# icdm-adteam/MoCoPCI

Hardware: AMD Instinct MI355X
Metric: interpolated frames/sec (higher is better)
Workload: dtype f32 (fused MLP layers: fp32 products as 6 bf16-MFMA partials of an exact 3-way split, fp32 accumulate; index paths exact f32)

## Files before the change

mocopci_amd/csrc/attention.hip:

```cpp
#include "attention_wide_fwd.h"

namespace {

typedef mcp_f2 f2;
constexpr int KT = 64;

template <int HD>
__global__ __launch_bounds__(64 * WAVES) void attention_small_kernel(int nq, int nk, int heads, const float *__restrict__ q, int qs,
                                                                     const float *__restrict__ k, int ks, const float *__restrict__ v,
                                                                     int vs, float scale_log2e, float *__restrict__ out, int os, int kv_shift) {
    constexpr int KS = HD + 1;
    __shared__ float kt[2][KT * KS];
    __shared__ __attribute__((aligned(16))) float vt[2][KT * HD];
    const int tid = threadIdx.x, lane = tid & 63, wave = tid >> 6, h = lane >> 5, col = lane & 31;
    const int head = blockIdx.y, bf = blockIdx.z;
    const int qi = blockIdx.x * (32 * WAVES) + wave * 32 + col;
    const bool live = qi < nq;
    q += ((size_t)bf * nq + (live ? qi : 0)) * qs + head * HD;
    int bkv = bf + kv_shift;
    if (bkv >= (int)gridDim.z) bkv -= (int)gridDim.z;
    k += (size_t)bkv * nk * ks + head * HD;
    v += (size_t)bkv * nk * vs + head * HD;

    float qf[HD / 2];
#pragma unroll
    for (int s = 0; s < HD / 2; ++s) qf[s] = q[2 * s + h] * scale_log2e;

    float m = -INFINITY, l = 0.f;
    f2 o[HD / 2];
#pragma unroll
    for (int d = 0; d < HD / 2; ++d) o[d] = f2{0.f, 0.f};

    constexpr int F4_PER_TILE = KT * HD / 4;
    constexpr int LOADS = (2 * F4_PER_TILE + 64 * WAVES - 1) / (64 * WAVES);
    float4 pre[LOADS];
    auto fetch = [&](int t) {
#pragma unroll
        for (int u = 0; u < LOADS; ++u) {
            const int e = tid + u * 64 * WAVES;
            const bool isv = e >= F4_PER_TILE;
            const int f = isv ? e - F4_PER_TILE : e;
            const int row = f / (HD / 4), c4 = f % (HD / 4);
            const int key = t * KT + row;
            pre[u] = make_float4(0.f, 0.f, 0.f, 0.f);
            if (e < 2 * F4_PER_TILE && key < nk) {
                const float *src = (isv ? v + (size_t)key * vs : k + (size_t)key * ks) + c4 * 4;
                pre[u] = *reinterpret_cast<const float4 *>(src);
            }
        }
    };
    auto stash = [&](int buf) {
#pragma unroll
        for (int u = 0; u < LOADS; ++u) {
            const int e = tid + u * 64 * WAVES;
            if (e >= 2 * F4_PER_TILE) continue;
            const bool isv = e >= F4_PER_TILE;
            const int f = isv ? e - F4_PER_TILE : e;
            const int row = f / (HD / 4), c4 = f % (HD / 4);
            if (isv) {
                *reinterpret_cast<float4 *>(&vt[buf][row * HD + c4 * 4]) = pre[u];
            } else {
                float *dst = &kt[buf][row * KS + c4 * 4];
                dst[0] = pre[u].x; dst[1] = pre[u].y; dst[2] = pre[u].z; dst[3] = pre[u].w;
            }
        }
    };

    const int stages = (nk + KT - 1) / KT;
    fetch(0);
    stash(0);
    for (int t = 0; t < stages; ++t) {
        const int cur = t & 1;
        if (t + 1 < stages) fetch(t + 1);
        __syncthreads();
#pragma unroll
        for (int sub = 0; sub < KT / 32; ++sub) {
            const float *ka = &kt[cur][(sub * 32 + col) * KS + h];
            f32x16 acc;
#pragma unroll
            for (int r = 0; r < 16; ++r) acc[r] = 0.f;
#pragma unroll
            for (int s = 0; s < HD / 2; ++s) acc = __builtin_amdgcn_mfma_f32_32x32x2f32(ka[2 * s], qf[s], acc, 0, 0, 0);
            const int kbase = t * KT + sub * 32;
            if (kbase + 32 > nk) {
#pragma unroll
                for (int r = 0; r < 16; ++r)
                    if (kbase + chan_of(r, h) >= nk) acc[r] = -INFINITY;
            }
            float mt = acc[0];
#pragma unroll
            for (int r = 1; r < 16; ++r) mt = fmaxf(mt, acc[r]);
            const float mn = fmaxf(m, mt);
            if (mn == -INFINITY) continue;
            const float alpha = __builtin_amdgcn_exp2f(m - mn);
            m = mn;
            l *= alpha;
            const f2 alpha2 = {alpha, alpha};
#pragma unroll
            for (int d = 0; d < HD / 2; ++d) o[d] = o[d] * alpha2;
#pragma unroll
            for (int r = 0; r < 16; ++r) {
                const float p = __builtin_amdgcn_exp2f(acc[r] - mn);
                l += p;
                const float *vr = &vt[cur][(sub * 32 + chan_of(r, h)) * HD];
                const f2 p2 = {p, p};
#pragma unroll
                for (int d = 0; d < HD; d += 4) {
                    const float4 vv = *reinterpret_cast<const float4 *>(vr + d);
                    o[d / 2 + 0] = mcp_f2_fma(p2, f2{vv.x, vv.y}, o[d / 2 + 0]);
                    o[d / 2 + 1] = mcp_f2_fma(p2, f2{vv.z, vv.w}, o[d / 2 + 1]);
                }
            }
        }
        if (t + 1 < stages) stash(cur ^ 1);
    }
    const float mo = __shfl_xor(m, 32), lo = __shfl_xor(l, 32);
    const float mm = fmaxf(m, mo);
    const float a0 = m == -INFINITY ? 0.f : __builtin_amdgcn_exp2f(m - mm), a1 = mo == -INFINITY ? 0.f : __builtin_amdgcn_exp2f(mo - mm);
    const float lsum = l * a0 + lo * a1;
    const float inv = 1.0f / lsum;
    float res[HD];
#pragma unroll
    for (int d = 0; d < HD; ++d) {
        const float od = (d & 1) ? o[d / 2].y : o[d / 2].x;
        res[d] = (od * a0 + __shfl_xor(od, 32) * a1) * inv;
    }
    if (live && h == 0) {
        float *dst = out + ((size_t)bf * nq + qi) * os + head * HD;
#pragma unroll
        for (int d = 0; d < HD; d += 4) *reinterpret_cast<float4 *>(dst + d) = make_float4(res[d], res[d + 1], res[d + 2], res[d + 3]);
    }
}

__device__ __forceinline__ int kv_batch(int kv_shift) {
    const int bkv = (int)blockIdx.z + kv_shift;
    return bkv >= (int)gridDim.z ? bkv - (int)gridDim.z : bkv;
}

template <int HD>
__global__ __launch_bounds__(64 * WAVES, 1) void attention_wide_kernel(int nq, int nk, const float *__restrict__ q, int qs,
                                                                       const float *__restrict__ k, int ks, const float *__restrict__ v,
                                                                       int vs, float scale_log2e, float *__restrict__ out, int os, int kv_shift) {
    extern __shared__ __attribute__((aligned(16))) float lds_w[];
    attention_wide_body<HD, false>(lds_w, nq, nk, (int)gridDim.y, q, qs, k, ks, v, vs, kv_batch(kv_shift), scale_log2e, 0, 0, 0.f, out, os, nullptr);
}

template <int HD>
__global__ __launch_bounds__(64 * WAVES, 1) void attention_wide_ksplit_kernel(int nq, int nk, const float *__restrict__ q, int qs,
                                                                              const float *__restrict__ k, int ks, const float *__restrict__ v,
                                                                              int vs, float scale_log2e, float *__restrict__ out, int os, int kv_shift) {
    extern __shared__ __attribute__((aligned(16))) float lds_ws[];
    attention_wide_ksplit_body<HD, false>(lds_ws, nq, nk, (int)gridDim.y, q, qs, k, ks, v, vs, kv_batch(kv_shift), scale_log2e, 0, 0, 0.f, out, os,
                                          nullptr);
}

template <int HD>
int launch_wide_ksplit(int bf, int nq, int nk, int heads, const float *q, int qs, const float *k, int ks, const float *v, int vs, float sl2,
                       float *out, int os, int kv_shift, hipStream_t s) {
    auto kern = attention_wide_ksplit_kernel<HD>;
    static McpPerDeviceOnce attr_once;
    if (attr_once.need()) {
        { const hipError_t attr_e_ = hipFuncSetAttribute(reinterpret_cast<const void *>(kern), hipFuncAttributeMaxDynamicSharedMemorySize, 160 * 1024); if (attr_e_ != hipSuccess) return (int)attr_e_; }
        attr_once.done();
    }
    hipLaunchKernelGGL(kern, dim3(mcp_divup(nq, 32), heads, bf), dim3(64 * WAVES), WideSplitCfg<HD>::LDS_BYTES, s, nq, nk, q, qs, k, ks, v, vs, sl2,
                       out, os, kv_shift);
    return mcp_launch_status();
}

template <int HD>
int launch_wide(int bf, int nq, int nk, int heads, const float *q, int qs, const float *k, int ks, const float *v, int vs, float sl2,
                float *out, int os, int kv_shift, hipStream_t s) {
    auto kern = attention_wide_kernel<HD>;
    static McpPerDeviceOnce attr_once;
    if (attr_once.need()) {
        { const hipError_t attr_e_ = hipFuncSetAttribute(reinterpret_cast<const void *>(kern), hipFuncAttributeMaxDynamicSharedMemorySize, 160 * 1024); if (attr_e_ != hipSuccess) return (int)attr_e_; }
        attr_once.done();
    }
    hipLaunchKernelGGL(kern, dim3(mcp_divup(nq, 32 * WAVES), heads, bf), dim3(64 * WAVES), WideCfg<HD>::LDS_BYTES, s, nq, nk, q, qs, k, ks, v,
                       vs, sl2, out, os, kv_shift);
    return mcp_launch_status();
}

}

namespace {
int attention_any(int bf, int nq, int nk, int heads, int hd, const float *q, int q_stride, const float *k, int k_stride, const float *v,
                  int v_stride, int kv_shift, float scale, float *out, int out_stride, hipStream_t s) {
    if (((uintptr_t)q | (uintptr_t)k | (uintptr_t)v | (uintptr_t)out) & 15) return MCP_ERR_BAD_ARG;
    if ((q_stride | k_stride | v_stride | out_stride) & 3) return MCP_ERR_BAD_ARG;
    if (kv_shift < 0 || kv_shift >= bf) return MCP_ERR_BAD_ARG;
    const float sl2 = scale * 1.44269504088896340736f;
    const dim3 grid(mcp_divup(nq, 32 * WAVES), heads, bf);
    int rc;
    mcp_prof_begin(MCP_KERNEL_ATTENTION, s);
    if (hd == 8 || hd == 16) {
        if (hd == 8)
            hipLaunchKernelGGL(attention_small_kernel<8>, grid, dim3(64 * WAVES), 0, s, nq, nk, heads, q, q_stride, k, k_stride, v, v_stride, sl2,
                               out, out_stride, kv_shift);
        else
            hipLaunchKernelGGL(attention_small_kernel<16>, grid, dim3(64 * WAVES), 0, s, nq, nk, heads, q, q_stride, k, k_stride, v, v_stride,
                               sl2, out, out_stride, kv_shift);
        rc = mcp_launch_status();
    } else {
        rc = hd == 32   ? launch_wide<32>(bf, nq, nk, heads, q, q_stride, k, k_stride, v, v_stride, sl2, out, out_stride, kv_shift, s)
             : hd == 64 ? launch_wide<64>(bf, nq, nk, heads, q, q_stride, k, k_stride, v, v_stride, sl2, out, out_stride, kv_shift, s)
                        : wide_keys_split(bf, nq, nk, heads)
                              ? launch_wide_ksplit<256>(bf, nq, nk, heads, q, q_stride, k, k_stride, v, v_stride, sl2, out, out_stride, kv_shift, s)
                              : launch_wide<256>(bf, nq, nk, heads, q, q_stride, k, k_stride, v, v_stride, sl2, out, out_stride, kv_shift, s);
    }
    mcp_prof_end(MCP_KERNEL_ATTENTION, s);
    return rc;
}
}

MCP_EXPORT int mcp_attention_small(int bf, int nq, int nk, int heads, int hd, const float *q, int q_stride, const float *k,
                                   int k_stride, const float *v, int v_stride, float scale, float *out, int out_stride,
                                   mcp_stream_t stream) {
    MCP_CHECK_ARGS(bf > 0 && nq > 0 && nk > 0 && heads > 0 && q && k && v && out);
    if (hd != 8 && hd != 16) return MCP_ERR_UNSUPPORTED;
    return attention_any(bf, nq, nk, heads, hd, q, q_stride, k, k_stride, v, v_stride, 0, scale, out, out_stride, (hipStream_t)stream);
}

MCP_EXPORT int mcp_attention_wide(int bf, int nq, int nk, int heads, int hd, const float *q, int q_stride, const float *k,
                                  int k_stride, const float *v, int v_stride, float scale, float *out, int out_stride,
                                  mcp_stream_t stream) {
    MCP_CHECK_ARGS(bf > 0 && nq > 0 && nk > 0 && heads > 0 && q && k && v && out);
    if (hd != 32 && hd != 64 && hd != 256) return MCP_ERR_UNSUPPORTED;
    return attention_any(bf, nq, nk, heads, hd, q, q_stride, k, k_stride, v, v_stride, 0, scale, out, out_stride, (hipStream_t)stream);
}

MCP_EXPORT int mcp_attention(int bf, int nq, int nk, int heads, int hd, const float *q, int q_stride, const float *k, int k_stride,
                             const float *v, int v_stride, int kv_batch_shift, float scale, float *out, int out_stride,
                             mcp_stream_t stream) {
    MCP_CHECK_ARGS(bf > 0 && nq > 0 && nk > 0 && heads > 0 && q && k && v && out);
    if (hd != 8 && hd != 16 && hd != 32 && hd != 64 && hd != 256) return MCP_ERR_UNSUPPORTED;
    return attention_any(bf, nq, nk, heads, hd, q, q_stride, k, k_stride, v, v_stride, kv_batch_shift, scale, out, out_stride,
                         (hipStream_t)stream);
}
```

mocopci_amd/csrc/attention_grad.hip:

```cpp
#include "common.h"
#include "attention_dropout.h"

namespace {

typedef float f32x16 __attribute__((ext_vector_type(16)));
constexpr int WAVES = 4, KT = 64;

__device__ __forceinline__ int chan_of(int r, int h) { return (r & 3) + 8 * (r >> 2) + 4 * h; }

template <int N>
__device__ __forceinline__ void pin(float (&a)[N]) {
#pragma unroll
    for (int i = 0; i < N; i += 8)
        asm volatile("" : "+v"(a[i]), "+v"(a[i + 1]), "+v"(a[i + 2]), "+v"(a[i + 3]), "+v"(a[i + 4]), "+v"(a[i + 5]), "+v"(a[i + 6]), "+v"(a[i + 7]));
}

template <int HD>
struct Stage {
    static constexpr int KS = HD + 1;
    static constexpr int PAD = KT * KS, PLAIN = KT * HD;
};

template <int HD, bool DROP>
__global__ __launch_bounds__(64 * WAVES) void attention_small_drop_kernel(int nq, int nk, int heads, const float *__restrict__ q, int qs,
                                                                          const float *__restrict__ k, int ks, const float *__restrict__ v, int vs,
                                                                          float scale_log2e, uint32_t seed, uint32_t threshold, float inv_keep,
                                                                          float *__restrict__ out, float *__restrict__ lse) {
    constexpr int KS = HD + 1;
    __shared__ float kt[2][KT * KS];
    __shared__ __attribute__((aligned(16))) float vt[2][KT * HD];
    const int tid = threadIdx.x, lane = tid & 63, wave = tid >> 6, h = lane >> 5, col = lane & 31;
    const int head = blockIdx.y, bf = blockIdx.z;
    const int qi = blockIdx.x * (32 * WAVES) + wave * 32 + col;
    const bool live = qi < nq;
    const size_t qrow = (size_t)bf * nq + (live ? qi : 0);
    const uint32_t row = (uint32_t)(((size_t)bf * heads + head) * nq + qi);
    q += qrow * qs + head * HD;
    k += (size_t)bf * nk * ks + head * HD;
    v += (size_t)bf * nk * vs + head * HD;
    float qf[HD / 2];
#pragma unroll
    for (int s = 0; s < HD / 2; ++s) qf[s] = q[2 * s + h] * scale_log2e;
    float m = -INFINITY, l = 0.f, o[HD];
#pragma unroll
    for (int d = 0; d < HD; ++d) o[d] = 0.f;
    constexpr int F4 = KT * HD / 4, LOADS = (2 * F4 + 64 * WAVES - 1) / (64 * WAVES);
    float4 pre[LOADS];
    auto fetch = [&](int t) {
#pragma unroll
        for (int u = 0; u < LOADS; ++u) {
            const int e = tid + u * 64 * WAVES;
            const bool isv = e >= F4;
            const int f = isv ? e - F4 : e, r_ = f / (HD / 4), c4 = f % (HD / 4), key = t * KT + r_;
            pre[u] = make_float4(0.f, 0.f, 0.f, 0.f);
            if (e < 2 * F4 && key < nk) pre[u] = *reinterpret_cast<const float4 *>((isv ? v + (size_t)key * vs : k + (size_t)key * ks) + c4 * 4);
        }
    };
    auto stash = [&](int buf) {
#pragma unroll
        for (int u = 0; u < LOADS; ++u) {
            const int e = tid + u * 64 * WAVES;
            if (e >= 2 * F4) continue;
            const bool isv = e >= F4;
            const int f = isv ? e - F4 : e, r_ = f / (HD / 4), c4 = f % (HD / 4);
            if (isv) {
                *reinterpret_cast<float4 *>(&vt[buf][r_ * HD + c4 * 4]) = pre[u];
            } else {
                float *dst = &kt[buf][r_ * KS + c4 * 4];
                dst[0] = pre[u].x; dst[1] = pre[u].y; dst[2] = pre[u].z; dst[3] = pre[u].w;
            }
        }
    };
    const int stages = (nk + KT - 1) / KT;
    fetch(0);
    stash(0);
    for (int t = 0; t < stages; ++t) {
        const int cur = t & 1;
        if (t + 1 < stages) fetch(t + 1);
        __syncthreads();
#pragma unroll
        for (int sub = 0; sub < KT / 32; ++sub) {
            const float *ka = &kt[cur][(sub * 32 + col) * KS + h];
            f32x16 acc;
#pragma unroll
            for (int r = 0; r < 16; ++r) acc[r] = 0.f;
#pragma unroll
            for (int s = 0; s < HD / 2; ++s) acc = __builtin_amdgcn_mfma_f32_32x32x2f32(ka[2 * s], qf[s], acc, 0, 0, 0);
            const int kbase = t * KT + sub * 32;
            if (kbase + 32 > nk) {
#pragma unroll
                for (int r = 0; r < 16; ++r)
                    if (kbase + chan_of(r, h) >= nk) acc[r] = -INFINITY;
            }
            float mt = acc[0];
#pragma unroll
            for (int r = 1; r < 16; ++r) mt = fmaxf(mt, acc[r]);
            const float mn = fmaxf(m, mt);
            if (mn == -INFINITY) continue;
            const float alpha = __builtin_amdgcn_exp2f(m - mn);
            m = mn;
            l *= alpha;
#pragma unroll
            for (int d = 0; d < HD; ++d) o[d] *= alpha;
#pragma unroll
            for (int r = 0; r < 16; ++r) {
                const float p = __builtin_amdgcn_exp2f(acc[r] - mn);
                l += p;
                float pm = DROP ? p * drop_scale(seed, row, (uint32_t)(kbase + chan_of(r, h)), threshold, inv_keep) : p;
                int off = (sub * 32 + chan_of(r, h)) * HD;
                asm volatile("" : "+v"(off), "+v"(pm));
                const float *vr = &vt[cur][off];
#pragma unroll
                for (int d = 0; d < HD; d += 4) {
                    const float4 vv = *reinterpret_cast<const float4 *>(vr + d);
                    o[d + 0] = __builtin_fmaf(pm, vv.x, o[d + 0]);
                    o[d + 1] = __builtin_fmaf(pm, vv.y, o[d + 1]);
                    o[d + 2] = __builtin_fmaf(pm, vv.z, o[d + 2]);
                    o[d + 3] = __builtin_fmaf(pm, vv.w, o[d + 3]);
                }
                pin(o);
            }
        }
        if (t + 1 < stages) stash(cur ^ 1);
    }
    const float mo = __shfl_xor(m, 32), lo = __shfl_xor(l, 32);
    const float mm = fmaxf(m, mo);
    const float a0 = m == -INFINITY ? 0.f : __builtin_amdgcn_exp2f(m - mm), a1 = mo == -INFINITY ? 0.f : __builtin_amdgcn_exp2f(mo - mm);
    const float lsum = l * a0 + lo * a1;
    const float inv = 1.0f / lsum;
    float res[HD];
#pragma unroll
    for (int d = 0; d < HD; ++d) res[d] = (o[d] * a0 + __shfl_xor(o[d], 32) * a1) * inv;
    if (live && h == 0) {
        float *dst = out + qrow * (size_t)(heads * HD) + head * HD;
#pragma unroll
        for (int d = 0; d < HD; d += 4) *reinterpret_cast<float4 *>(dst + d) = make_float4(res[d], res[d + 1], res[d + 2], res[d + 3]);
        if (lse) lse[((size_t)bf * heads + head) * nq + qi] = mm + __builtin_amdgcn_logf(lsum);
    }
}

template <int HD>
__global__ __launch_bounds__(256) void attention_dsum_kernel(long long rows, int heads, const float *__restrict__ out, const float *__restrict__ gout,
                                                            int nq, float *__restrict__ dsum) {
    const long long e = (long long)blockIdx.x * 256 + threadIdx.x;
    if (e >= rows) return;
    const float4 *o = reinterpret_cast<const float4 *>(out + e * HD), *g = reinterpret_cast<const float4 *>(gout + e * HD);
    float d = 0.f;
#pragma unroll
    for (int c = 0; c < HD / 4; ++c) {
        const float4 a = g[c], b = o[c];
        d = __builtin_fmaf(a.x, b.x, d); d = __builtin_fmaf(a.y, b.y, d); d = __builtin_fmaf(a.z, b.z, d); d = __builtin_fmaf(a.w, b.w, d);
    }
    const long long bq = e / heads;
    const int head = (int)(e - bq * heads);
    const long long bfi = bq / nq;
    const int qi = (int)(bq - bfi * nq);
    dsum[(bfi * heads + head) * nq + qi] = d;
}

template <int HD>
__global__ __launch_bounds__(64 * WAVES) void attention_stats_kernel(int nq, int nk, int heads, const float *__restrict__ q, int qs, const float *__restrict__ k,
                                                                     int ks, float scale_log2e, const float *__restrict__ out, const float *__restrict__ gout,
                                                                     float *__restrict__ lse, float *__restrict__ dsum) {
    constexpr int KS = HD + 1;
    __shared__ float kt[2][KT * KS];
    const int tid = threadIdx.x, lane = tid & 63, wave = tid >> 6, h = lane >> 5, col = lane & 31;
    const int head = blockIdx.y, bf = blockIdx.z;
    const int qi = blockIdx.x * (32 * WAVES) + wave * 32 + col;
    const bool live = qi < nq;
    const size_t qrow = (size_t)bf * nq + (live ? qi : 0);
    q += qrow * qs + head * HD;
    k += (size_t)bf * nk * ks + head * HD;
    float qf[HD / 2];
#pragma unroll
    for (int s = 0; s < HD / 2; ++s) qf[s] = q[2 * s + h] * scale_log2e;
    float m = -INFINITY, l = 0.f;
    constexpr int F4 = KT * HD / 4, LOADS = (F4 + 64 * WAVES - 1) / (64 * WAVES);
    float4 pre[LOADS];
    auto fetch = [&](int t) {
#pragma unroll
        for (int u = 0; u < LOADS; ++u) {
            const int e = tid + u * 64 * WAVES, row = e / (HD / 4), c4 = e % (HD / 4), key = t * KT + row;
            pre[u] = make_float4(0.f, 0.f, 0.f, 0.f);
            if (e < F4 && key < nk) pre[u] = *reinterpret_cast<const float4 *>(k + (size_t)key * ks + c4 * 4);
        }
    };
    auto stash = [&](int buf) {
#pragma unroll
        for (int u = 0; u < LOADS; ++u) {
            const int e = tid + u * 64 * WAVES, row = e / (HD / 4), c4 = e % (HD / 4);
            if (e >= F4) continue;
            float *dst = &kt[buf][row * KS + c4 * 4];
            dst[0] = pre[u].x; dst[1] = pre[u].y; dst[2] = pre[u].z; dst[3] = pre[u].w;
        }
    };
    const int stages = (nk + KT - 1) / KT;
    fetch(0);
    stash(0);
    for (int t = 0; t < stages; ++t) {
        const int cur = t & 1;
        if (t + 1 < stages) fetch(t + 1);
        __syncthreads();
#pragma unroll
        for (int sub = 0; sub < KT / 32; ++sub) {
            const float *ka = &kt[cur][(sub * 32 + col) * KS + h];
            f32x16 acc;
#pragma unroll
            for (int r = 0; r < 16; ++r) acc[r] = 0.f;
#pragma unroll
            for (int s = 0; s < HD / 2; ++s) acc = __builtin_amdgcn_mfma_f32_32x32x2f32(ka[2 * s], qf[s], acc, 0, 0, 0);
            const int kbase = t * KT + sub * 32;
            if (kbase + 32 > nk) {
#pragma unroll
                for (int r = 0; r < 16; ++r)
                    if (kbase + chan_of(r, h) >= nk) acc[r] = -INFINITY;
            }
            float mt = acc[0];
#pragma unroll
            for (int r = 1; r < 16; ++r) mt = fmaxf(mt, acc[r]);
            const float mn = fmaxf(m, mt);
            if (mn == -INFINITY) continue;
            l *= __builtin_amdgcn_exp2f(m - mn);
            m = mn;
#pragma unroll
            for (int r = 0; r < 16; ++r) l += __builtin_amdgcn_exp2f(acc[r] - mn);
        }
        if (t + 1 < stages) stash(cur ^ 1);
    }
    const float mo = __shfl_xor(m, 32), lo = __shfl_xor(l, 32);
    const float mm = fmaxf(m, mo);
    const float a0 = m == -INFINITY ? 0.f : __builtin_amdgcn_exp2f(m - mm), a1 = mo == -INFINITY ? 0.f : __builtin_amdgcn_exp2f(mo - mm);
    const float lsum = l * a0 + lo * a1;
    if (live && h == 0) {
        const float *orow = out + qrow * (size_t)(heads * HD) + head * HD, *grow = gout + qrow * (size_t)(heads * HD) + head * HD;
        float d = 0.f;
#pragma unroll
        for (int c = 0; c < HD; ++c) d = __builtin_fmaf(grow[c], orow[c], d);
        const size_t o = ((size_t)bf * heads + head) * nq + qi;
        lse[o] = mm + __builtin_amdgcn_logf(lsum);
        dsum[o] = d;
    }
}

template <int HD, bool DROP>
__global__ __launch_bounds__(64 * WAVES, 2) void attention_dq_kernel(int nq, int nk, int heads, const float *__restrict__ q, int qs, const float *__restrict__ k,
                                                                  int ks, const float *__restrict__ v, int vs, float scale_log2e, float scale,
                                                                  uint32_t seed, uint32_t threshold, float inv_keep,
                                                                  const float *__restrict__ gout, const float *__restrict__ lse,
                                                                  const float *__restrict__ dsum, float *__restrict__ dq) {
    constexpr int KS = HD + 1;
    __shared__ float kt[2][KT * KS];
    __shared__ float vt[2][KT * KS];
    __shared__ __attribute__((aligned(16))) float kp[2][KT * HD];
    const int tid = threadIdx.x, lane = tid & 63, wave = tid >> 6, h = lane >> 5, col = lane & 31;
    const int head = blockIdx.y, bf = blockIdx.z;
    const int qi = blockIdx.x * (32 * WAVES) + wave * 32 + col;
    const bool live = qi < nq;
    const size_t qrow = (size_t)bf * nq + (live ? qi : 0);
    q += qrow * qs + head * HD;
    k += (size_t)bf * nk * ks + head * HD;
    v += (size_t)bf * nk * vs + head * HD;
    const float *grow = gout + qrow * (size_t)(heads * HD) + head * HD;
    const size_t so = ((size_t)bf * heads + head) * nq + (live ? qi : 0);
    const float L = lse[so], D = dsum[so];
    const uint32_t drow = (uint32_t)(((size_t)bf * heads + head) * nq + qi);
    float qf[HD / 2], gf[HD / 2];
#pragma unroll
    for (int s = 0; s < HD / 2; ++s) {
        qf[s] = q[2 * s + h] * scale_log2e;
        gf[s] = grow[2 * s + h];
    }
    float acc_q[HD];
#pragma unroll
    for (int d = 0; d < HD; ++d) acc_q[d] = 0.f;
    constexpr int F4 = KT * HD / 4, LOADS = (2 * F4 + 64 * WAVES - 1) / (64 * WAVES);
    float4 pre[LOADS];
    auto fetch = [&](int t) {
#pragma unroll
        for (int u = 0; u < LOADS; ++u) {
            const int e = tid + u * 64 * WAVES;
            const bool isv = e >= F4;
            const int f = isv ? e - F4 : e, row = f / (HD / 4), c4 = f % (HD / 4), key = t * KT + row;
            pre[u] = make_float4(0.f, 0.f, 0.f, 0.f);
            if (e < 2 * F4 && key < nk) pre[u] = *reinterpret_cast<const float4 *>((isv ? v + (size_t)key * vs : k + (size_t)key * ks) + c4 * 4);
        }
    };
    auto stash = [&](int buf) {
#pragma unroll
        for (int u = 0; u < LOADS; ++u) {
            const int e = tid + u * 64 * WAVES;
            if (e >= 2 * F4) continue;
            const bool isv = e >= F4;
            const int f = isv ? e - F4 : e, row = f / (HD / 4), c4 = f % (HD / 4);
            float *dst = isv ? &vt[buf][row * KS + c4 * 4] : &kt[buf][row * KS + c4 * 4];
            dst[0] = pre[u].x; dst[1] = pre[u].y; dst[2] = pre[u].z; dst[3] = pre[u].w;
            if (!isv) *reinterpret_cast<float4 *>(&kp[buf][row * HD + c4 * 4]) = pre[u];
        }
    };
    const int stages = (nk + KT - 1) / KT;
    fetch(0);
    stash(0);
    for (int t = 0; t < stages; ++t) {
        const int cur = t & 1;
        if (t + 1 < stages) fetch(t + 1);
        __syncthreads();
#pragma unroll
        for (int sub = 0; sub < KT / 32; ++sub) {
            const float *ka = &kt[cur][(sub * 32 + col) * KS + h], *va = &vt[cur][(sub * 32 + col) * KS + h];
            f32x16 acc, accp;
#pragma unroll
            for (int r = 0; r < 16; ++r) { acc[r] = 0.f; accp[r] = 0.f; }
#pragma unroll
            for (int s = 0; s < HD / 2; ++s) {
                acc = __builtin_amdgcn_mfma_f32_32x32x2f32(ka[2 * s], qf[s], acc, 0, 0, 0);
                accp = __builtin_amdgcn_mfma_f32_32x32x2f32(va[2 * s], gf[s], accp, 0, 0, 0);
            }
            const int kbase = t * KT + sub * 32;
#pragma unroll
            for (int r = 0; r < 16; ++r) {
                const int key = sub * 32 + chan_of(r, h);
                float p = __builtin_amdgcn_exp2f(acc[r] - L);
                if (kbase + chan_of(r, h) >= nk) p = 0.f;
                const float mk = DROP ? drop_scale(seed, drow, (uint32_t)(kbase + chan_of(r, h)), threshold, inv_keep) : 1.0f;
                float ds = p * (mk * accp[r] - D);
                int off = key * HD;
                asm volatile("" : "+v"(off), "+v"(ds));
                const float *kr = &kp[cur][off];
#pragma unroll
                for (int d = 0; d < HD; d += 4) {
                    const float4 kk = *reinterpret_cast<const float4 *>(kr + d);
                    acc_q[d + 0] = __builtin_fmaf(ds, kk.x, acc_q[d + 0]);
                    acc_q[d + 1] = __builtin_fmaf(ds, kk.y, acc_q[d + 1]);
                    acc_q[d + 2] = __builtin_fmaf(ds, kk.z, acc_q[d + 2]);
                    acc_q[d + 3] = __builtin_fmaf(ds, kk.w, acc_q[d + 3]);
                }
                pin(acc_q);
            }
        }
        if (t + 1 < stages) stash(cur ^ 1);
    }
    float res[HD];
#pragma unroll
    for (int d = 0; d < HD; ++d) res[d] = (acc_q[d] + __shfl_xor(acc_q[d], 32)) * scale;
    if (live && h == 0) {
        float *dst = dq + qrow * (size_t)(heads * HD) + head * HD;
#pragma unroll
        for (int d = 0; d < HD; d += 4) *reinterpret_cast<float4 *>(dst + d) = make_float4(res[d], res[d + 1], res[d + 2], res[d + 3]);
    }
}

template <int HD, bool DROP>
__global__ __launch_bounds__(64 * WAVES, 2) void attention_dkv_kernel(int nq, int nk, int heads, const float *__restrict__ q, int qs, const float *__restrict__ k,
                                                                   int ks, const float *__restrict__ v, int vs, float scale_log2e, float scale,
                                                                   uint32_t seed, uint32_t threshold, float inv_keep,
                                                                   const float *__restrict__ gout, const float *__restrict__ lse,
                                                                   const float *__restrict__ dsum, float *__restrict__ dkv) {
    constexpr int KS = HD + 1;
    __shared__ float qt[2][KT * KS];
    __shared__ float gt[2][KT * KS];
    __shared__ __attribute__((aligned(16))) float qp[2][KT * HD];
    __shared__ __attribute__((aligned(16))) float gp[2][KT * HD];
    __shared__ float lt[2][KT], dt[2][KT];
    const int tid = threadIdx.x, lane = tid & 63, wave = tid >> 6, h = lane >> 5, col = lane & 31;
    const int head = blockIdx.y, bf = blockIdx.z;
    const int ki = blockIdx.x * (32 * WAVES) + wave * 32 + col;
    const bool live = ki < nk;
    const size_t krow = (size_t)bf * nk + (live ? ki : 0);
    const float *kr_ = k + krow * ks + head * HD, *vr_ = v + krow * vs + head * HD;
    q += (size_t)bf * nq * qs + head * HD;
    gout += (size_t)bf * nq * (size_t)(heads * HD) + head * HD;
    lse += ((size_t)bf * heads + head) * nq;
    dsum += ((size_t)bf * heads + head) * nq;
    const uint32_t rbase = (uint32_t)(((size_t)bf * heads + head) * nq);
    float kf[HD / 2], vf[HD / 2];
#pragma unroll
    for (int s = 0; s < HD / 2; ++s) {
        kf[s] = kr_[2 * s + h] * scale_log2e;
        vf[s] = vr_[2 * s + h];
    }
    float acc_k[HD], acc_v[HD];
#pragma unroll
    for (int d = 0; d < HD; ++d) { acc_k[d] = 0.f; acc_v[d] = 0.f; }
    constexpr int F4 = KT * HD / 4, LOADS = (2 * F4 + 64 * WAVES - 1) / (64 * WAVES);
    float4 pre[LOADS];
    float pl = 0.f, pd = 0.f;
    auto fetch = [&](int t) {
#pragma unroll
        for (int u = 0; u < LOADS; ++u) {
            const int e = tid + u * 64 * WAVES;
            const bool isg = e >= F4;
            const int f = isg ? e - F4 : e, row = f / (HD / 4), c4 = f % (HD / 4), qq = t * KT + row;
            pre[u] = make_float4(0.f, 0.f, 0.f, 0.f);
            if (e < 2 * F4 && qq < nq) pre[u] = *reinterpret_cast<const float4 *>((isg ? gout + (size_t)qq * (heads * HD) : q + (size_t)qq * qs) + c4 * 4);
        }
        if (tid < KT) {
            const int qq = t * KT + tid;
            pl = qq < nq ? lse[qq] : INFINITY;
            pd = qq < nq ? dsum[qq] : 0.f;
        }
    };
    auto stash = [&](int buf) {
#pragma unroll
        for (int u = 0; u < LOADS; ++u) {
            const int e = tid + u * 64 * WAVES;
            if (e >= 2 * F4) continue;
            const bool isg = e >= F4;
            const int f = isg ? e - F4 : e, row = f / (HD / 4), c4 = f % (HD / 4);
            float *dst = isg ? &gt[buf][row * KS + c4 * 4] : &qt[buf][row * KS + c4 * 4];
            dst[0] = pre[u].x; dst[1] = pre[u].y; dst[2] = pre[u].z; dst[3] = pre[u].w;
            *reinterpret_cast<float4 *>(isg ? &gp[buf][row * HD + c4 * 4] : &qp[buf][row * HD + c4 * 4]) = pre[u];
        }
        if (tid < KT) {
            lt[buf][tid] = pl;
            dt[buf][tid] = pd;
        }
    };
    const int stages = (nq + KT - 1) / KT;
    fetch(0);
    stash(0);
    for (int t = 0; t < stages; ++t) {
        const int cur = t & 1;
        if (t + 1 < stages) fetch(t + 1);
        __syncthreads();
#pragma unroll
        for (int sub = 0; sub < KT / 32; ++sub) {
            const float *qa = &qt[cur][(sub * 32 + col) * KS + h], *ga = &gt[cur][(sub * 32 + col) * KS + h];
            f32x16 acc, accp;
#pragma unroll
            for (int r = 0; r < 16; ++r) { acc[r] = 0.f; accp[r] = 0.f; }
#pragma unroll
            for (int s = 0; s < HD / 2; ++s) {
                acc = __builtin_amdgcn_mfma_f32_32x32x2f32(qa[2 * s], kf[s], acc, 0, 0, 0);
                accp = __builtin_amdgcn_mfma_f32_32x32x2f32(ga[2 * s], vf[s], accp, 0, 0, 0);
            }
#pragma unroll
            for (int r = 0; r < 16; ++r) {
                const int qq = sub * 32 + chan_of(r, h);
                const float p = __builtin_amdgcn_exp2f(acc[r] - lt[cur][qq]);
                const float mk = DROP ? drop_scale(seed, rbase + (uint32_t)(t * KT + qq), (uint32_t)ki, threshold, inv_keep) : 1.0f;
                const float pm = DROP ? p * mk : p;
                float ds = p * (mk * accp[r] - dt[cur][qq]);
// ... 155 lines not shown
```

Before: 3678.

## Move small-head attention P·V accumulation onto 4x4 MFMA and share forward body

The small-head-dim (8/16) attention kernels now accumulate P·V with mfma_f32_4x4x1f32 instead of per-lane VALU FMAs over float4 V rows from LDS. This aims to offload the inner accumulation loop to the matrix units and cut LDS reads and VALU work. The code is factored into a shared header used by both the inference and dropout/LSE kernels. It also adds amdgpu_waves_per_eu occupancy hints, a branchless fully-masked-tile path and a sched_barrier per sub-tile. The MFMA lane mapping is subtle and could hurt accuracy or performance if it misbehaves. The old FMA path stays available under an A/B compile flag and environment variable.

```diff
diff --git a/mocopci_amd/csrc/attention.hip b/mocopci_amd/csrc/attention.hip
--- a/mocopci_amd/csrc/attention.hip
+++ b/mocopci_amd/csrc/attention.hip
@@ -1,136 +1,33 @@
+#include <stdlib.h>
+
 #include "attention_wide_fwd.h"
+#include "attention_small_fwd.h"
 
 namespace {
 
-typedef mcp_f2 f2;
-constexpr int KT = 64;
-
 template <int HD>
-__global__ __launch_bounds__(64 * WAVES) void attention_small_kernel(int nq, int nk, int heads, const float *__restrict__ q, int qs,
+__global__ __launch_bounds__(64 * WAVES) __attribute__((amdgpu_waves_per_eu(SmallCfg<HD>::OCC))) void attention_small_kernel(int nq, int nk, int heads, const float *__restrict__ q, int qs,
                                                                      const float *__restrict__ k, int ks, const float *__restrict__ v,
                                                                      int vs, float scale_log2e, float *__restrict__ out, int os, int kv_shift) {
-    constexpr int KS = HD + 1;
-    __shared__ float kt[2][KT * KS];
-    __shared__ __attribute__((aligned(16))) float vt[2][KT * HD];
-    const int tid = threadIdx.x, lane = tid & 63, wave = tid >> 6, h = lane >> 5, col = lane & 31;
-    const int head = blockIdx.y, bf = blockIdx.z;
-    const int qi = blockIdx.x * (32 * WAVES) + wave * 32 + col;
-    const bool live = qi < nq;
-    q += ((size_t)bf * nq + (live ? qi : 0)) * qs + head * HD;
-    int bkv = bf + kv_shift;
+    __shared__ float kt[SmallCfg<HD>::K_FLOATS];
+    __shared__ __attribute__((aligned(16))) float vt[SmallCfg<HD>::V_FLOATS];
+    int bkv = (int)blockIdx.z + kv_shift;
     if (bkv >= (int)gridDim.z) bkv -= (int)gridDim.z;
-    k += (size_t)bkv * nk * ks + head * HD;
-    v += (size_t)bkv * nk * vs + head * HD;
+    attention_small_body<HD, false, true>(kt, vt, nq, nk, heads, q, qs, k, ks, v, vs, bkv, scale_log2e, 0, 0, 0.f, out, os, nullptr);
+}
 
-    float qf[HD / 2];
-#pragma unroll
-    for (int s = 0; s < HD / 2; ++s) qf[s] = q[2 * s + h] * scale_log2e;
-
-    float m = -INFINITY, l = 0.f;
-    f2 o[HD / 2];
-#pragma unroll
-    for (int d = 0; d < HD / 2; ++d) o[d] = f2{0.f, 0.f};
-
-    constexpr int F4_PER_TILE = KT * HD / 4;
-    constexpr int LOADS = (2 * F4_PER_TILE + 64 * WAVES - 1) / (64 * WAVES);
-    float4 pre[LOADS];
-    auto fetch = [&](int t) {
-#pragma unroll
-        for (int u = 0; u < LOADS; ++u) {
-            const int e = tid + u * 64 * WAVES;
-            const bool isv = e >= F4_PER_TILE;
-            const int f = isv ? e - F4_PER_TILE : e;
-            const int row = f / (HD / 4), c4 = f % (HD / 4);
-            const int key = t * KT + row;
-            pre[u] = make_float4(0.f, 0.f, 0.f, 0.f);
-            if (e < 2 * F4_PER_TILE && key < nk) {
-                const float *src = (isv ? v + (size_t)key * vs : k + (size_t)key * ks) + c4 * 4;
-                pre[u] = *reinterpret_cast<const float4 *>(src);
-            }
-        }
-    };
-    auto stash = [&](int buf) {
-#pragma unroll
-        for (int u = 0; u < LOADS; ++u) {
-            const int e = tid + u * 64 * WAVES;
-            if (e >= 2 * F4_PER_TILE) continue;
-            const bool isv = e >= F4_PER_TILE;
-            const int f = isv ? e - F4_PER_TILE : e;
-            const int row = f / (HD / 4), c4 = f % (HD / 4);
-            if (isv) {
-                *reinterpret_cast<float4 *>(&vt[buf][row * HD + c4 * 4]) = pre[u];
-            } else {
-                float *dst = &kt[buf][row * KS + c4 * 4];
-                dst[0] = pre[u].x; dst[1] = pre[u].y; dst[2] = pre[u].z; dst[3] = pre[u].w;
-            }
-        }
-    };
-
-    const int stages = (nk + KT - 1) / KT;
-    fetch(0);
-    stash(0);
-    for (int t = 0; t < stages; ++t) {
-        const int cur = t & 1;
-        if (t + 1 < stages) fetch(t + 1);
-        __syncthreads();
-#pragma unroll
-        for (int sub = 0; sub < KT / 32; ++sub) {
-            const float *ka = &kt[cur][(sub * 32 + col) * KS + h];
-            f32x16 acc;
-#pragma unroll
-            for (int r = 0; r < 16; ++r) acc[r] = 0.f;
-#pragma unroll
-            for (int s = 0; s < HD / 2; ++s) acc = __builtin_amdgcn_mfma_f32_32x32x2f32(ka[2 * s], qf[s], acc, 0, 0, 0);
-            const int kbase = t * KT + sub * 32;
-            if (kbase + 32 > nk) {
-#pragma unroll
-                for (int r = 0; r < 16; ++r)
-                    if (kbase + chan_of(r, h) >= nk) acc[r] = -INFINITY;
-            }
-            float mt = acc[0];
-#pragma unroll
-            for (int r = 1; r < 16; ++r) mt = fmaxf(mt, acc[r]);
-            const float mn = fmaxf(m, mt);
-            if (mn == -INFINITY) continue;
-            const float alpha = __builtin_amdgcn_exp2f(m - mn);
-            m = mn;
-            l *= alpha;
-            const f2 alpha2 = {alpha, alpha};
-#pragma unroll
-            for (int d = 0; d < HD / 2; ++d) o[d] = o[d] * alpha2;
-#pragma unroll
-            for (int r = 0; r < 16; ++r) {
-                const float p = __builtin_amdgcn_exp2f(acc[r] - mn);
-                l += p;
-                const float *vr = &vt[cur][(sub * 32 + chan_of(r, h)) * HD];
-                const f2 p2 = {p, p};
-#pragma unroll
-                for (int d = 0; d < HD; d += 4) {
-                    const float4 vv = *reinterpret_cast<const float4 *>(vr + d);
-                    o[d / 2 + 0] = mcp_f2_fma(p2, f2{vv.x, vv.y}, o[d / 2 + 0]);
-                    o[d / 2 + 1] = mcp_f2_fma(p2, f2{vv.z, vv.w}, o[d / 2 + 1]);
-                }
-            }
-        }
-        if (t + 1 < stages) stash(cur ^ 1);
-    }
-    const float mo = __shfl_xor(m, 32), lo = __shfl_xor(l, 32);
-    const float mm = fmaxf(m, mo);
-    const float a0 = m == -INFINITY ? 0.f : __builtin_amdgcn_exp2f(m - mm), a1 = mo == -INFINITY ? 0.f : __builtin_amdgcn_exp2f(mo - mm);
-    const float lsum = l * a0 + lo * a1;
-    const float inv = 1.0f / lsum;
-    float res[HD];
-#pragma unroll
-    for (int d = 0; d < HD; ++d) {
-        const float od = (d & 1) ? o[d / 2].y : o[d / 2].x;
-        res[d] = (od * a0 + __shfl_xor(od, 32) * a1) * inv;
-    }
-    if (live && h == 0) {
-        float *dst = out + ((size_t)bf * nq + qi) * os + head * HD;
-#pragma unroll
-        for (int d = 0; d < HD; d += 4) *reinterpret_cast<float4 *>(dst + d) = make_float4(res[d], res[d + 1], res[d + 2], res[d + 3]);
-    }
+#ifdef MCP_AB
+template <int HD>
+__global__ __launch_bounds__(64 * WAVES) void attention_small_fma_kernel(int nq, int nk, int heads, const float *__restrict__ q, int qs,
+                                                                         const float *__restrict__ k, int ks, const float *__restrict__ v,
+                                                                         int vs, float scale_log2e, float *__restrict__ out, int os, int kv_shift) {
+    __shared__ float kt[SmallCfg<HD>::K_FLOATS];
+    __shared__ __attribute__((aligned(16))) float vt[SmallCfg<HD>::V_FLOATS];
+    int bkv = (int)blockIdx.z + kv_shift;
+    if (bkv >= (int)gridDim.z) bkv -= (int)gridDim.z;
+    attention_small_body<HD, false, false>(kt, vt, nq, nk, heads, q, qs, k, ks, v, vs, bkv, scale_log2e, 0, 0, 0.f, out, os, nullptr);
 }
+#endif
 
 __device__ __forceinline__ int kv_batch(int kv_shift) {
     const int bkv = (int)blockIdx.z + kv_shift;
@@ -195,6 +92,16 @@
     int rc;
     mcp_prof_begin(MCP_KERNEL_ATTENTION, s);
     if (hd == 8 || hd == 16) {
+#ifdef MCP_AB
+        static const bool pv_fma = [] { const char *e = getenv("MCP_ATTENTION_PV_FMA"); return e && *e == '1'; }();
+        if (pv_fma && hd == 8)
+            hipLaunchKernelGGL(attention_small_fma_kernel<8>, grid, dim3(64 * WAVES), 0, s, nq, nk, heads, q, q_stride, k, k_stride, v, v_stride, sl2,
+                               out, out_stride, kv_shift);
+        else if (pv_fma)
+            hipLaunchKernelGGL(attention_small_fma_kernel<16>, grid, dim3(64 * WAVES), 0, s, nq, nk, heads, q, q_stride, k, k_stride, v, v_stride,
+                               sl2, out, out_stride, kv_shift);
+        else
+#endif
         if (hd == 8)
             hipLaunchKernelGGL(attention_small_kernel<8>, grid, dim3(64 * WAVES), 0, s, nq, nk, heads, q, q_stride, k, k_stride, v, v_stride, sl2,
                                out, out_stride, kv_shift);
diff --git a/mocopci_amd/csrc/attention_grad.hip b/mocopci_amd/csrc/attention_grad.hip
--- a/mocopci_amd/csrc/attention_grad.hip
+++ b/mocopci_amd/csrc/attention_grad.hip
@@ -1,5 +1,6 @@
 #include "common.h"
 #include "attention_dropout.h"
+#include "attention_small_fwd.h"
 
 namespace {
 
@@ -22,121 +23,15 @@
 };
 
 template <int HD, bool DROP>
-__global__ __launch_bounds__(64 * WAVES) void attention_small_drop_kernel(int nq, int nk, int heads, const float *__restrict__ q, int qs,
+__global__ __launch_bounds__(64 * WAVES) __attribute__((amdgpu_waves_per_eu(DROP ? SmallCfg<HD>::OCC_DROP : SmallCfg<HD>::OCC_LSE)))
+void attention_small_drop_kernel(int nq, int nk, int heads, const float *__restrict__ q, int qs,
                                                                           const float *__restrict__ k, int ks, const float *__restrict__ v, int vs,
                                                                           float scale_log2e, uint32_t seed, uint32_t threshold, float inv_keep,
                                                                           float *__restrict__ out, float *__restrict__ lse) {
-    constexpr int KS = HD + 1;
-    __shared__ float kt[2][KT * KS];
-    __shared__ __attribute__((aligned(16))) float vt[2][KT * HD];
-    const int tid = threadIdx.x, lane = tid & 63, wave = tid >> 6, h = lane >> 5, col = lane & 31;
-    const int head = blockIdx.y, bf = blockIdx.z;
-    const int qi = blockIdx.x * (32 * WAVES) + wave * 32 + col;
-    const bool live = qi < nq;
-    const size_t qrow = (size_t)bf * nq + (live ? qi : 0);
-    const uint32_t row = (uint32_t)(((size_t)bf * heads + head) * nq + qi);
-    q += qrow * qs + head * HD;
-    k += (size_t)bf * nk * ks + head * HD;
-    v += (size_t)bf * nk * vs + head * HD;
-    float qf[HD / 2];
-#pragma unroll
-    for (int s = 0; s < HD / 2; ++s) qf[s] = q[2 * s + h] * scale_log2e;
-    float m = -INFINITY, l = 0.f, o[HD];
-#pragma unroll
-    for (int d = 0; d < HD; ++d) o[d] = 0.f;
-    constexpr int F4 = KT * HD / 4, LOADS = (2 * F4 + 64 * WAVES - 1) / (64 * WAVES);
-    float4 pre[LOADS];
-    auto fetch = [&](int t) {
-#pragma unroll
-        for (int u = 0; u < LOADS; ++u) {
-            const int e = tid + u * 64 * WAVES;
-            const bool isv = e >= F4;
-            const int f = isv ? e - F4 : e, r_ = f / (HD / 4), c4 = f % (HD / 4), key = t * KT + r_;
-            pre[u] = make_float4(0.f, 0.f, 0.f, 0.f);
-            if (e < 2 * F4 && key < nk) pre[u] = *reinterpret_cast<const float4 *>((isv ? v + (size_t)key * vs : k + (size_t)key * ks) + c4 * 4);
-        }
-    };
-    auto stash = [&](int buf) {
-#pragma unroll
-        for (int u = 0; u < LOADS; ++u) {
-            const int e = tid + u * 64 * WAVES;
-            if (e >= 2 * F4) continue;
-            const bool isv = e >= F4;
-            const int f = isv ? e - F4 : e, r_ = f / (HD / 4), c4 = f % (HD / 4);
-            if (isv) {
-                *reinterpret_cast<float4 *>(&vt[buf][r_ * HD + c4 * 4]) = pre[u];
-            } else {
-                float *dst = &kt[buf][r_ * KS + c4 * 4];
-                dst[0] = pre[u].x; dst[1] = pre[u].y; dst[2] = pre[u].z; dst[3] = pre[u].w;
-            }
-        }
-    };
-    const int stages = (nk + KT - 1) / KT;
-    fetch(0);
-    stash(0);
-    for (int t = 0; t < stages; ++t) {
-        const int cur = t & 1;
-        if (t + 1 < stages) fetch(t + 1);
-        __syncthreads();
-#pragma unroll
-        for (int sub = 0; sub < KT / 32; ++sub) {
-            const float *ka = &kt[cur][(sub * 32 + col) * KS + h];
-            f32x16 acc;
-#pragma unroll
-            for (int r = 0; r < 16; ++r) acc[r] = 0.f;
-#pragma unroll
-            for (int s = 0; s < HD / 2; ++s) acc = __builtin_amdgcn_mfma_f32_32x32x2f32(ka[2 * s], qf[s], acc, 0, 0, 0);
-            const int kbase = t * KT + sub * 32;
-            if (kbase + 32 > nk) {
-#pragma unroll
-                for (int r = 0; r < 16; ++r)
-                    if (kbase + chan_of(r, h) >= nk) acc[r] = -INFINITY;
-            }
-            float mt = acc[0];
-#pragma unroll
-            for (int r = 1; r < 16; ++r) mt = fmaxf(mt, acc[r]);
-            const float mn = fmaxf(m, mt);
-            if (mn == -INFINITY) continue;
-            const float alpha = __builtin_amdgcn_exp2f(m - mn);
-            m = mn;
-            l *= alpha;
-#pragma unroll
-            for (int d = 0; d < HD; ++d) o[d] *= alpha;
-#pragma unroll
-            for (int r = 0; r < 16; ++r) {
-                const float p = __builtin_amdgcn_exp2f(acc[r] - mn);
-                l += p;
-                float pm = DROP ? p * drop_scale(seed, row, (uint32_t)(kbase + chan_of(r, h)), threshold, inv_keep) : p;
-                int off = (sub * 32 + chan_of(r, h)) * HD;
-                asm volatile("" : "+v"(off), "+v"(pm));
-                const float *vr = &vt[cur][off];
-#pragma unroll
-                for (int d = 0; d < HD; d += 4) {
-                    const float4 vv = *reinterpret_cast<const float4 *>(vr + d);
-                    o[d + 0] = __builtin_fmaf(pm, vv.x, o[d + 0]);
-                    o[d + 1] = __builtin_fmaf(pm, vv.y, o[d + 1]);
-                    o[d + 2] = __builtin_fmaf(pm, vv.z, o[d + 2]);
-                    o[d + 3] = __builtin_fmaf(pm, vv.w, o[d + 3]);
-                }
-                pin(o);
-            }
-        }
-        if (t + 1 < stages) stash(cur ^ 1);
-    }
-    const float mo = __shfl_xor(m, 32), lo = __shfl_xor(l, 32);
-    const float mm = fmaxf(m, mo);
-    const float a0 = m == -INFINITY ? 0.f : __builtin_amdgcn_exp2f(m - mm), a1 = mo == -INFINITY ? 0.f : __builtin_amdgcn_exp2f(mo - mm);
-    const float lsum = l * a0 + lo * a1;
-    const float inv = 1.0f / lsum;
-    float res[HD];
-#pragma unroll
-    for (int d = 0; d < HD; ++d) res[d] = (o[d] * a0 + __shfl_xor(o[d], 32) * a1) * inv;
-    if (live && h == 0) {
-        float *dst = out + qrow * (size_t)(heads * HD) + head * HD;
-#pragma unroll
-        for (int d = 0; d < HD; d += 4) *reinterpret_cast<float4 *>(dst + d) = make_float4(res[d], res[d + 1], res[d + 2], res[d + 3]);
-        if (lse) lse[((size_t)bf * heads + head) * nq + qi] = mm + __builtin_amdgcn_logf(lsum);
-    }
+    __shared__ float kt[SmallCfg<HD>::K_FLOATS];
+    __shared__ __attribute__((aligned(16))) float vt[SmallCfg<HD>::V_FLOATS];
+    attention_small_body<HD, DROP, true>(kt, vt, nq, nk, heads, q, qs, k, ks, v, vs, (int)blockIdx.z, scale_log2e, seed, threshold, inv_keep, out,
+                                         heads * HD, lse);
 }
 
 template <int HD>
diff --git a/mocopci_amd/csrc/attention_small_fwd.h b/mocopci_amd/csrc/attention_small_fwd.h
--- /dev/null
+++ b/mocopci_amd/csrc/attention_small_fwd.h
@@ -0,0 +1,174 @@
+#pragma once
+#include "common.h"
+#include "attention_dropout.h"
+
+namespace {
+
+typedef float small_f32x16 __attribute__((ext_vector_type(16)));
+typedef float small_f32x4 __attribute__((ext_vector_type(4)));
+
+template <int HD>
+struct SmallCfg {
+    static constexpr int WAVES = 4;
+    static constexpr int KT = 64;
+    static constexpr int KS = HD + 1;
+    static constexpr int K_FLOATS = 2 * KT * KS, V_FLOATS = 2 * KT * HD;
+    static constexpr int OCC = HD == 8 ? 7 : 4, OCC_LSE = HD == 8 ? 6 : 4, OCC_DROP = 4;
+};
+
+__device__ __forceinline__ int small_key_of(int r, int h) { return (r & 3) + 8 * (r >> 2) + 4 * h; }
+
+template <int HD, bool DROP, bool MFMA>
+__device__ __forceinline__ void attention_small_tile(small_f32x16 acc, const float *vrows, int kbase, int nk, int h, int lane, float &m, float &l,
+                                                     float (&o)[HD], uint32_t seed, uint32_t row, uint32_t threshold, float inv_keep) {
+    if (kbase + 32 > nk) {
+#pragma unroll
+        for (int r = 0; r < 16; ++r)
+            if (kbase + small_key_of(r, h) >= nk) acc[r] = -INFINITY;
+    }
+    float mt = acc[0];
+#pragma unroll
+    for (int r = 1; r < 16; ++r) mt = fmaxf(mt, acc[r]);
+    const float mn = fmaxf(m, mt);
+    const bool seen = mn != -INFINITY;
+    const float ms = seen ? mn : 0.f;
+    const float alpha = seen ? __builtin_amdgcn_exp2f(m - ms) : 1.f;
+    m = mn;
+    l *= alpha;
+#pragma unroll
+    for (int d = 0; d < HD; ++d) o[d] *= alpha;
+    if (MFMA) {
+        small_f32x4 og[HD / 4];
+#pragma unroll
+        for (int g = 0; g < HD / 4; ++g) og[g] = small_f32x4{o[4 * g], o[4 * g + 1], o[4 * g + 2], o[4 * g + 3]};
+        const float *va = vrows + (lane & 3);
+#pragma unroll
+        for (int r = 0; r < 16; ++r) {
+            const float p = __builtin_amdgcn_exp2f(acc[r] - ms);
+            l += p;
+            const float pm = DROP ? p * drop_scale(seed, row, (uint32_t)(kbase + small_key_of(r, h)), threshold, inv_keep) : p;
+            const float *vr = va + small_key_of(r, h) * HD;
+#pragma unroll
+            for (int g = 0; g < HD / 4; ++g) og[g] = __builtin_amdgcn_mfma_f32_4x4x1f32(vr[4 * g], pm, og[g], 0, 0, 0);
+        }
+#pragma unroll
+        for (int g = 0; g < HD / 4; ++g) {
+            o[4 * g] = og[g][0]; o[4 * g + 1] = og[g][1]; o[4 * g + 2] = og[g][2]; o[4 * g + 3] = og[g][3];
+        }
+    } else {
+#pragma unroll
+        for (int r = 0; r < 16; ++r) {
+            const float p = __builtin_amdgcn_exp2f(acc[r] - ms);
+            l += p;
+            const float pm = DROP ? p * drop_scale(seed, row, (uint32_t)(kbase + small_key_of(r, h)), threshold, inv_keep) : p;
+            const float *vr = vrows + small_key_of(r, h) * HD;
+#pragma unroll
+            for (int d = 0; d < HD; d += 4) {
+                const float4 vv = *reinterpret_cast<const float4 *>(vr + d);
+                o[d + 0] = __builtin_fmaf(pm, vv.x, o[d + 0]);
+                o[d + 1] = __builtin_fmaf(pm, vv.y, o[d + 1]);
+                o[d + 2] = __builtin_fmaf(pm, vv.z, o[d + 2]);
+                o[d + 3] = __builtin_fmaf(pm, vv.w, o[d + 3]);
+            }
+        }
+    }
+}
+
+template <int HD, bool DROP, bool MFMA>
+__device__ __forceinline__ void attention_small_body(float *kt, float *vt, int nq, int nk, int heads, const float *__restrict__ q, int qs,
+                                                     const float *__restrict__ k, int ks, const float *__restrict__ v, int vs, int bkv,
+                                                     float scale_log2e, uint32_t seed, uint32_t threshold, float inv_keep,
+                                                     float *__restrict__ out, int os, float *__restrict__ lse) {
+    using C = SmallCfg<HD>;
+    constexpr int WAVES = C::WAVES, KT = C::KT, KS = C::KS;
+    const int tid = threadIdx.x, lane = tid & 63, wave = tid >> 6, h = lane >> 5, col = lane & 31;
+    const int head = blockIdx.y, bf = blockIdx.z;
+    const int qi = blockIdx.x * (32 * WAVES) + wave * 32 + col;
+    const bool live = qi < nq;
+    const size_t qrow = (size_t)bf * nq + (live ? qi : 0);
+    const uint32_t row = (uint32_t)(((size_t)bf * heads + head) * nq + qi);
+    q += qrow * qs + head * HD;
+    k += (size_t)bkv * nk * ks + head * HD;
+    v += (size_t)bkv * nk * vs + head * HD;
+
+    float qf[HD / 2];
+#pragma unroll
+    for (int s = 0; s < HD / 2; ++s) qf[s] = q[2 * s + h] * scale_log2e;
+
+    float m = -INFINITY, l = 0.f, o[HD];
+#pragma unroll
+    for (int d = 0; d < HD; ++d) o[d] = 0.f;
+
+    constexpr int F4_PER_TILE = KT * HD / 4;
+    constexpr int LOADS = (2 * F4_PER_TILE + 64 * WAVES - 1) / (64 * WAVES);
+    float4 pre[LOADS];
+    auto fetch = [&](int t) {
+#pragma unroll
+        for (int u = 0; u < LOADS; ++u) {
+            const int e = tid + u * 64 * WAVES;
+            const bool isv = e >= F4_PER_TILE;
+            const int f = isv ? e - F4_PER_TILE : e;
+            const int r_ = f / (HD / 4), c4 = f % (HD / 4);
+            const int key = t * KT + r_;
+            pre[u] = make_float4(0.f, 0.f, 0.f, 0.f);
+            if (e < 2 * F4_PER_TILE && key < nk) {
+                const float *src = (isv ? v + (size_t)key * vs : k + (size_t)key * ks) + c4 * 4;
+                pre[u] = *reinterpret_cast<const float4 *>(src);
+            }
+        }
+    };
+    auto stash = [&](int buf) {
+#pragma unroll
+        for (int u = 0; u < LOADS; ++u) {
+            const int e = tid + u * 64 * WAVES;
+            if (e >= 2 * F4_PER_TILE) continue;
+            const bool isv = e >= F4_PER_TILE;
+            const int f = isv ? e - F4_PER_TILE : e;
+            const int r_ = f / (HD / 4), c4 = f % (HD / 4);
+            if (isv) {
+                *reinterpret_cast<float4 *>(&vt[buf * (KT * HD) + r_ * HD + c4 * 4]) = pre[u];
+            } else {
+                float *dst = &kt[buf * (KT * KS) + r_ * KS + c4 * 4];
+                dst[0] = pre[u].x; dst[1] = pre[u].y; dst[2] = pre[u].z; dst[3] = pre[u].w;
+            }
+        }
+    };
+
+    const int stages = (nk + KT - 1) / KT;
+    fetch(0);
+    stash(0);
+    for (int t = 0; t < stages; ++t) {
+        const int cur = t & 1;
+        if (t + 1 < stages) fetch(t + 1);
+        __syncthreads();
+#pragma unroll
+        for (int sub = 0; sub < KT / 32; ++sub) {
+            const float *ka = &kt[cur * (KT * KS) + (sub * 32 + col) * KS + h];
+            small_f32x16 acc;
+#pragma unroll
+            for (int r = 0; r < 16; ++r) acc[r] = 0.f;
+#pragma unroll
+            for (int s = 0; s < HD / 2; ++s) acc = __builtin_amdgcn_mfma_f32_32x32x2f32(ka[2 * s], qf[s], acc, 0, 0, 0);
+            attention_small_tile<HD, DROP, MFMA>(acc, &vt[cur * (KT * HD) + sub * 32 * HD], t * KT + sub * 32, nk, h, lane, m, l, o, seed, row, threshold,
+                                                 inv_keep);
+            __builtin_amdgcn_sched_barrier(0);
+        }
+        if (t + 1 < stages) stash(cur ^ 1);
+    }
+    const float mo = __shfl_xor(m, 32), lo = __shfl_xor(l, 32);
+    const float mm = fmaxf(m, mo);
+    const float a0 = m == -INFINITY ? 0.f : __builtin_amdgcn_exp2f(m - mm), a1 = mo == -INFINITY ? 0.f : __builtin_amdgcn_exp2f(mo - mm);
+    const float lsum = l * a0 + lo * a1;
+    const float inv = 1.0f / lsum;
+    float res[HD];
+#pragma unroll
+    for (int d = 0; d < HD; ++d) res[d] = (o[d] * a0 + __shfl_xor(o[d], 32) * a1) * inv;
+    if (live && h == 0) {
+        float *dst = out + qrow * (size_t)os + head * HD;
+#pragma unroll
+        for (int d = 0; d < HD; d += 4) *reinterpret_cast<float4 *>(dst + d) = make_float4(res[d], res[d + 1], res[d + 2], res[d + 3]);
+        if (lse) lse[((size_t)bf * heads + head) * nq + qi] = mm + __builtin_amdgcn_logf(lsum);
+    }
+}
+
+}
```

Result: no change. 3655 (-0.6%).
